# RajeshRk18/exacto

Hardware: AMD Instinct MI355X
Metric: ciphertext muls/sec (bfv_mul_and_relin) (higher is better)
Workload: dtype u64; 1 GPU; bfv_mul_and_relin, BASELINE configs[2]; ring_degree=4096, ct_limbs=3, limb_bits=60, plain_modulus=65537, gadget_base=65536, gadget_digits=12, batch_per_gpu=1024, global_batch=1024, parallelism=batch-shard x1

## Files before the change

### exacto_amd/csrc/context.hip

```cpp
#include <algorithm>
#include <array>
#include <cxxabi.h>
#include <dlfcn.h>
#include <chrono>
#include <condition_variable>
#include <cmath>
#include <cstdio>
#include <cstdlib>
#include <cstring>
#include <functional>
#include <map>
#include <memory>
#include <mutex>
#include <set>
#include <string>
#include <thread>
#include <type_traits>
#include <vector>

#include "../../include/exacto_hip.h"
#include "exacto_internal.hpp"

using namespace exacto;

// ... 3054 lines not shown


extern "C" int exacto_gen_galois_key_dev(exacto_ctx* c, const uint64_t* sk, uint64_t element, double sigma,
                                         const uint64_t* key, uint64_t stream, size_t num_keys, uint64_t* gk) {
    if (int e = check_ctx(c)) return e;
    if (!key || !sk || !gk) return invalid_param("null argument");
    if (num_keys == 0) return 0;
    const int n = c->n, L = c->L;
    const long Ln = (long)L * n;
    if (c->enc_buf.grow((size_t)(2 * n + Ln) * sizeof(u64))) return EXACTO_ERR_HIP;
    u64 *t0 = c->enc_buf, *t1 = t0 + n, *s_auto = t1 + n;
    HIP_TRY(dev_copy(t0, sk, n * sizeof(u64), c->stream));
    if (int e = run_ntt(c, contiguous(t0, 1, 1, 0, 1, n), 1, true)) return e;
    launch_automorph(t0, n, t1, n, 1, 1, n, 1, element, c->d_primes, 0, c->stream);
    launch_lift_q0(t1, s_auto, 1, n, L, c->d_primes, c->stream);
    CHECK_LAUNCH();
    if (int e = ntt_items(c, s_auto, 1, 0, L)) return e;
    std::vector<u64> gpow(num_keys * L);
    for (int l = 0; l < L; ++l) {
        const u64 q = c->primes[l];
        u64 g = 1 % q;
        const u64 b = c->gbase % q;
        for (size_t i = 0; i < num_keys; ++i) {
            gpow[i * L + l] = g;
            g = (u64)((u128)g * b % q);
        }
    }
    if (c->d_gpow.grow(gpow.size() * sizeof(u64))) return EXACTO_ERR_HIP;
    HIP_TRY(hipStreamSynchronize(c->stream));
    if (int e_ = upload(c, c->d_gpow, gpow.data(), gpow.size() * sizeof(u64))) return e_;
    const ChaChaKey k = chacha_key(key);
    if (int e = sample_polys(c, KG_UNIFORM, k, stream, gk + Ln, 2 * Ln, 0, 2, (long)num_keys, sigma)) return e;
    if (int e = sample_polys(c, KG_GAUSSIAN, k, stream, gk, 2 * Ln, 1, 2, (long)num_keys, sigma)) return e;
    if (int e = ntt_items(c, gk, (long)num_keys, 2 * Ln, 2L * L)) return e;
    launch_combine(KG_GALOIS, gk, (long)num_keys, 2 * Ln, Ln, sk, s_auto, nullptr, nullptr, c->d_gpow, n, L,
                   c->d_primes, c->stream);
    CHECK_LAUNCH();
    HIP_TRY(hipStreamSynchronize(c->stream));
    return 0;
}

extern "C" int exacto_bfv_apply_automorphism_dev(exacto_ctx* c, const uint64_t* ct, size_t polys, uint64_t element,
                                                 const uint64_t* gk, size_t num_keys, uint64_t* out, size_t B) {
    if (int e = check_ctx(c)) return e;
    if (polys != 2) return invalid_param("automorphism requires degree-1 ciphertext");
    if (num_keys == 0 || !gk) return invalid_param("galois key is empty");
    if (B == 0) return 0;
    const int n = c->n, L = c->L;
    const long Ln = (long)L * n;
    const int guse = (int)std::min<size_t>(c->G, num_keys);
    const size_t count = (size_t)guse * 2 * Ln;
    const bool d16 = c->digit16 && c->gbase <= 65536;
    const Ks32Basis& kb = c->kn;
    const bool k32 = d16 && c->ks32 && kb.S > 0 && c->path == EXACTO_PATH_EXACT_RNS;
    if (k32) {
        if (int e = ks32_convert_key(c, gk, (size_t)guse, c->d_gk_rs, kb.S, kb.d_p32, kb.mac_form)) return e;
    } else {
        if (c->gk_s.grow(count * sizeof(u64))) return EXACTO_ERR_HIP;
        launch_shoup_companions(gk, c->gk_s, (long)count, n, L, c->d_primes, c->stream);
        CHECK_LAUNCH();
    }
    const size_t C = std::min<size_t>(c->chunk, B);
    LanePass pass;
    if (int e = pass.begin(c, (long)((B + C - 1) / C), C)) return e;
    for (size_t s0 = 0; s0 < B; s0 += C) {
        const int cnt = (int)std::min(C, B - s0);
        LaneGuard lane = pass.chunk((long)(s0 / C));
        const u64* src = ct + s0 * 2 * Ln;
        u64* dst = out + s0 * 2 * Ln;
        NttBatch nb{};
        nb.src = src; nb.src_item_stride = 2 * Ln;
        nb.dst = c->ws.coefQ; nb.dst_item_stride = 2 * Ln;
        nb.ppi = 2 * L; nb.prime_base = 0; nb.period = L;
        if (int e = run_ntt(c, nb, (long)cnt * 2 * L, true)) return e;
        launch_automorph(c->ws.coefQ, 2 * Ln, c->ws.T, 2 * Ln, cnt, 2, n, L, element, c->d_primes, -1, c->stream);
        CHECK_LAUNCH();
        if (k32) {
            launch_decompose(c->ws.T + Ln, 2 * Ln, c->ws.D, guse, cnt, n, c->d_crt, c->d_primes, L, c->stream,
                             c->ws.D16);
            CHECK_LAUNCH();
            launch_rows(c->ws.T + Ln, 2 * Ln, nullptr, 0, Ln, cnt, c->stream);
            CHECK_LAUNCH();
            ks32_digits(c->ws.D16, c->ws.DS, cnt, guse, kb.S, c->logn, kb.d_p32, kb.mac_form, c->stream);
            ks32_mac(c->ws.DS, c->d_gk_rs, c->ws.U, cnt, guse, L, kb.S, n, kb.d_p32, kb.mac_form, c->stream);
            ks32_crt(c->ws.U, c->ws.T, 2 * Ln, cnt, L, kb.S, c->logn, kb.d_kst, kb.d_p32, c->d_primes, kb.mac_form, c->stream,
                     c->ks_fpc && kb.fpc_max >= 1);
            CHECK_LAUNCH();
            NttBatch rb{};
            rb.src = c->ws.T; rb.src_item_stride = 2 * Ln;
            rb.dst = dst; rb.dst_item_stride = 2 * Ln;
            rb.ppi = 2 * L; rb.prime_base = 0; rb.period = L;
            if (int e = run_ntt(c, rb, (long)cnt * 2 * L, false)) return e;
            continue;
        }
        NttBatch c0{};
        c0.src = c->ws.T; c0.src_item_stride = 2 * Ln;
        c0.dst = dst; c0.dst_item_stride = 2 * Ln;
        c0.ppi = L; c0.prime_base = 0; c0.period = L;
        if (int e = run_ntt(c, c0, (long)cnt * L, false)) return e;
        launch_rows(dst + Ln, 2 * Ln, nullptr, 0, Ln, cnt, c->stream);
        launch_decompose(c->ws.T + Ln, 2 * Ln, c->ws.D, guse, cnt, n, c->d_crt, c->d_primes, L, c->stream,
                         d16 ? c->ws.D16 : nullptr);
        CHECK_LAUNCH();
        NttBatch db = contiguous(c->ws.D, cnt, (long)guse * L, 0, L, n);
        if (d16) {
            db.src16 = c->ws.D16;
            db.src16_item_stride = (long)guse * n;
        }
        if (int e = run_ntt(c, db, (long)cnt * guse * L, false)) return e;
        launch_relin_mac(dst, 2 * Ln, c->ws.D, gk, c->gk_s, guse, dst, 2 * Ln, cnt, n, L, c->d_primes, c->stream);
        CHECK_LAUNCH();
    }
    return 0;
}

extern "C" int exacto_gen_galois_key(exacto_ctx* c, const uint64_t* sk, uint64_t element, double sigma,
                                     const uint64_t* key, uint64_t stream, size_t num_keys, uint64_t* gk) {
    if (!c) return invalid_param("null context");
    return host_call(c, {{sk, c->L * poly_bytes(c)}}, num_keys * 2 * c->L * poly_bytes(c), gk,
                     [&](std::vector<u64*>& d, u64* o) {
                         return exacto_gen_galois_key_dev(c, d[0], element, sigma, key, stream, num_keys, o);
                     });
}

extern "C" int exacto_bfv_apply_automorphism(exacto_ctx* c, const uint64_t* ct, size_t polys, uint64_t element,
                                             const uint64_t* gk, size_t num_keys, uint64_t* out, size_t B) {
    if (!c) return invalid_param("null context");
    if (polys != 2) return invalid_param("automorphism requires degree-1 ciphertext");
    return host_call(c, {{ct, B * 2 * c->L * poly_bytes(c)}, {gk, num_keys * 2 * c->L * poly_bytes(c)}},
                     B * 2 * c->L * poly_bytes(c), out, [&](std::vector<u64*>& d, u64* o) {
                         return exacto_bfv_apply_automorphism_dev(c, d[0], polys, element, d[1], num_keys, o, B);
                     });
}


static int pl_scratch(exacto_ctx* c, size_t words) {
    if (c->pl_buf.grow(words * sizeof(u64))) return EXACTO_ERR_HIP;
    return 0;
}

static int lift_plain(exacto_ctx* c, const u64* pt, long items, bool delta) {
    const long Ln = (long)c->L * c->n;
    if (delta)
        if (int e = delta_residues(c)) return e;
    if (int e = pl_scratch(c, (size_t)items * Ln)) return e;
    launch_scale_plain(pt, delta ? c->d_delta : nullptr, c->pl_buf, items, c->n, c->L, c->d_primes, c->stream);
    CHECK_LAUNCH();
    return ntt_items(c, c->pl_buf, items, Ln, c->L);
}

extern "C" int exacto_bfv_plain_mul_dev(exacto_ctx* c, const uint64_t* ct, size_t polys, const uint64_t* pt,
                                        uint64_t* out, size_t B) {
    if (int e = check_ctx(c)) return e;
    if (!ct || !pt || !out) return invalid_param("null argument");
    if (polys == 0) return invalid_param("ciphertext has no components");
    if (B == 0) return 0;
    if (int e = lift_plain(c, pt, (long)B, false)) return e;
    const long Ln = (long)c->L * c->n;
    launch_plain_apply(PLAIN_MUL, ct, (long)polys * Ln, out, (long)B, (int)polys, c->pl_buf, Ln, c->n, c->L, c->d_primes,
                       c->stream);
    CHECK_LAUNCH();
    return 0;
}

extern "C" int exacto_bfv_plain_add_dev(exacto_ctx* c, const uint64_t* ct, size_t polys, const uint64_t* pt,
                                        uint64_t* out, size_t B) {
    if (int e = check_ctx(c)) return e;
// ... 2227 lines not shown
```

### exacto_amd/csrc/exacto_internal.hpp

```cpp
#pragma once
#include "arith.hpp"

namespace exacto {

struct NttBatch {
    const u64* src;
    const u64* src_off;
    long src_item_stride;
    u64* dst;
    long dst_item_stride;
    int ppi;
    int prime_base;
    int period;
    const int16_t* src16;
    long src16_item_stride;
    int lazy_out;
};

enum class MulPath : int { Exact = 0, Hps = 1 };

struct CrtTables {
    int L;
    int K;
    int G;
    int gshift;
    u64 gbase;
    u64 plain;
    u64 gq_w[EXACTO_MAX_L][EXACTO_MAX_L];
    u64 gq_ws[EXACTO_MAX_L][EXACTO_MAX_L];
    u64 halfQ_mr[EXACTO_MAX_L];
    u64 qpref_w[EXACTO_MAX_L + 1][EXACTO_MAX_PRIMES];
    u64 qpref_ws[EXACTO_MAX_L + 1][EXACTO_MAX_PRIMES];
    u64 gp_w[EXACTO_MAX_K][EXACTO_MAX_K];
    u64 gp_ws[EXACTO_MAX_K][EXACTO_MAX_K];
    u64 halfP_mr[EXACTO_MAX_K];
    u64 ppref_w[EXACTO_MAX_K + 1][EXACTO_MAX_L];
    u64 ppref_ws[EXACTO_MAX_K + 1][EXACTO_MAX_L];
    u64 qinvp_w[EXACTO_MAX_K], qinvp_ws[EXACTO_MAX_K];
    u64 pq_w[EXACTO_MAX_K], pq_ws[EXACTO_MAX_K];
    u64 qpq_w[EXACTO_MAX_L + 1][EXACTO_MAX_K], qpq_ws[EXACTO_MAX_L + 1][EXACTO_MAX_K];
    u64 fpc_pq[EXACTO_MAX_K];
    u64 fpc_qpq[EXACTO_MAX_L][EXACTO_MAX_K];
    u64 fpc_neg[EXACTO_MAX_K];
    double fpc_inv[EXACTO_MAX_K];
    u64 fpc_pm[EXACTO_MAX_K][EXACTO_MAX_L];
    u64 fpc_negP[EXACTO_MAX_L];
    u64 fpq_pz_w[EXACTO_MAX_L], fpq_pz_ws[EXACTO_MAX_L];
    double fpq_inv0[EXACTO_MAX_L], fpq_inv1[EXACTO_MAX_L];
    u64 fpq_c[EXACTO_MAX_L][EXACTO_MAX_K];
    u64 fpq_qo_w[EXACTO_MAX_L], fpq_qo_ws[EXACTO_MAX_L];
    int near;
    int fast;
    int special;
    int digit_small;
    u64 pmod_w[EXACTO_MAX_PRIMES], pmod_ws[EXACTO_MAX_PRIMES];
    u64 Qwords[EXACTO_MAX_L];
    u64 hq[EXACTO_MAX_PRIMES];
    u64 hps_qinv[2];
    u64 hps_p1_inv_p0, hps_p0_inv_p1;
    u64 hps_pc;
    u64 hps_qinv_s[2];
    u64 hps_t_w[2], hps_t_ws[2];
    u64 hps_pq_w[2], hps_pq_ws[2];
    u64 hps_kPq[3];
    u64 hps_P[2], hps_halfP[2];
};

bool launch_ntt_fwd2(const NttBatch& nb1, int count1, const NttBatch& nb2, int count2, int logn,
                     const PrimeConst* primes, hipStream_t s);
void launch_ntt(const NttBatch& nb, int count, int logn, bool inverse, bool lazy, const PrimeConst* primes,
                hipStream_t s, bool asm_fwd = false, bool asm_inv = false, int qbits = 64);

void launch_shoup_companions(const u64* w, u64* ws, long count, int n, int L, const PrimeConst* primes,
                             hipStream_t s);

#define EXACTO_KS32_MAXS 4
struct Prime32 {
    uint32_t p;
    uint32_t n_inv, n_inv_s;
    uint32_t last_w, last_ws;
    uint32_t c32, c32s;
    uint32_t k63;
    uint32_t fn_inv, fn_inv_s;
    uint32_t flast_w, flast_ws;
    double inv_p;
    const uint2* tw_fwd;
    const uint2* tw_inv;
};
struct Ks32Tables {
    uint32_t ginv[EXACTO_KS32_MAXS][EXACTO_KS32_MAXS];
    uint32_t ginv_s[EXACTO_KS32_MAXS][EXACTO_KS32_MAXS];
    uint32_t halfP[EXACTO_KS32_MAXS];
    u64 pref_w[EXACTO_MAX_L][EXACTO_KS32_MAXS];
    u64 pref_ws[EXACTO_MAX_L][EXACTO_KS32_MAXS];
    u64 negP[EXACTO_MAX_L];
    uint32_t fpc_c[EXACTO_MAX_L][EXACTO_KS32_MAXS][2];
    uint32_t fpc_n[EXACTO_MAX_L][2];
};
void ks32_digits(const int16_t* D16, uint32_t* DS, int items, int G, int S, int logn, const Prime32* primes,
                 int form, hipStream_t st);
void ks32_digits32(const int32_t* D, uint32_t* DS, int items, int G, int S, int logn, const Prime32* primes,
                   int form, hipStream_t st);
void ks32_key(const u64* K, uint32_t* RS, long rows, int L, int S, int logn, const Prime32* primes,
              const PrimeConst* qprimes, int form, hipStream_t st);
void ks32_key_norms(const u64* K, u64* out, long rows, int L, int n, const PrimeConst* qprimes, hipStream_t st);
void ks32_mac(const uint32_t* DS, const uint32_t* RS, uint32_t* U, int items, int G, int L, int S, int n,
              const Prime32* primes, int mac_form, hipStream_t st);
void ks32_mac_hoist(const uint32_t* DS, const uint32_t* RSK, uint32_t* U, const uint32_t* perm,
                    const unsigned char* ident, int items, int R, int G, int L, int S, int n, const Prime32* primes,
                    int mac_form, hipStream_t st);
void ks32_crt(const uint32_t* U, u64* R, long r_stride, int items, int L, int S, int logn, const Ks32Tables* KT,
              const Prime32* primes, const PrimeConst* qprimes, int form, hipStream_t st, bool fpc = false);

struct BatchTab {
    Prime32 P;
    u64 mu;
    const uint32_t* perm;
};
enum { BF_STRICT = 3 };
void launch_batch_transform(bool encode, const u64* in, u64* out, long count, int logn, const BatchTab& tab, int form,
                            hipStream_t s);
void launch_dbfv_batch(bool encode, const u64* in, u64* out, long count, int d, u64 base, u64 p, int logn,
                       const BatchTab& tab, int form, hipStream_t s);

struct Operands {
    const u64* a;
    const u64* a_off;
    long a_stride;
    const u64* b;
    const u64* b_off;
    long b_stride;
    const u64* ea;
    const u64* ea_off;
    const u64* eb;
    const u64* eb_off;
};

bool launch_polymul(const u64* A, const u64* B, u64* out, long rows, int period, int logn, const PrimeConst* primes,
                    hipStream_t s);
void launch_mul_inv(const u64* A, const u64* B, u64* out, long rows, int period, int logn, bool lazy, bool asm_inv,
                    const PrimeConst* primes, hipStream_t s);
struct DropPrimeK {
    u64 w[EXACTO_MAX_L], ws[EXACTO_MAX_L];
};
void launch_drop_prime(const u64* in, u64* out, long rows, int l, bool round, const DropPrimeK& C, int logn, bool lazy,
                       bool asm_rounds, const PrimeConst* primes, hipStream_t s);
void launch_inv_tensor(const Operands& op, const u64* extP, u64* T, int items, int logn, int L, int K, bool lazy,
                       const PrimeConst* primes, hipStream_t s, bool asm_inv = false, bool p2only = false,
                       int qbits = 64, int share_np = 0, bool lazy_out = false, bool fold = false,
                       bool square = false);
bool crt_fold_tensor_ok(int logn, bool asm_inv, bool lazy_out);
void launch_phase(const u64* ct, int polys, long ct_stride, const u64* sk, u64* out, int items, int n, int L,
                  const PrimeConst* primes, hipStream_t s);
void launch_decrypt_round(const u64* X, u64* out, int items, int n, int L, const CrtTables* ct,
                          const PrimeConst* primes, u64 plain, hipStream_t s);
int noise_chunks(int n);
void launch_noise(const u64* X, const u64* expected, u64* plain_out, u64* part, u64* out, long items, int group,
                  int n, int L, const CrtTables* ct, const PrimeConst* primes, const u64* delta, u64 plain,
                  bool round, hipStream_t s);
void launch_dbfv_recompose(const u64* digits, u64* out, int items, int n, int d, u64 base, u64 plain, u64 t,
                           bool scalar, hipStream_t s);
void launch_exact_lift(const u64* coefQ, u64* extP, long rows, int n, const CrtTables* ct,
                       const PrimeConst* primes, int L, int K, int mode, hipStream_t s);
void launch_hps_extend(const u64* coefQ, u64* extP, long rows, int n, const PrimeConst* primes,
                       int K, hipStream_t s);
bool exact_scale_sp_ok(int L, int K, int mode);
void launch_exact_scale(const u64* T, u64* R, long r_stride, int ncomp_r, u64* D, int16_t* D16, int guse,
                        int items, int n, const CrtTables* ct, const PrimeConst* primes, int L,
                        int K, int mode, hipStream_t s, int gshift = -1, bool c2only = false,
                        bool digits8 = false, bool fpc = false, double fpq_lim = 0.0, bool fold = false);
bool exact_scale_fold_ok(int L, int K, int mode, bool fpc, double fpq_lim);
void launch_hps_scale(const u64* T, u64* R, long r_stride, int ncomp_r, u64* D, void* D16, bool d8, int guse,
                      int items, int n, const CrtTables* ct, const PrimeConst* primes, int K, bool fast,
                      hipStream_t s);
void launch_decompose(const u64* C2, long c2_stride, u64* D, int guse, int items, int n,
                      const CrtTables* ct, const PrimeConst* primes, int L, hipStream_t s, int16_t* D16 = nullptr);
void launch_rows(u64* dst, long dst_stride, const u64* src, long src_stride, long len, long rows, hipStream_t s);
void launch_copy_u64(u64* dst, const u64* src, long words, hipStream_t s);
void launch_xcd_probe(const u64* src, u64* dst, long words, uint32_t* xcc, int blocks, hipStream_t s);
void launch_fill_u32(uint32_t* dst, uint32_t v, long words, hipStream_t s);
void debug_watch_set(const void* lo, const void* hi, uint32_t* hit, hipStream_t s = nullptr);
void launch_relin_mac(const u64* base, long base_stride, const u64* D, const u64* rlk, const u64* rlk_s,
                      int guse, u64* out, long out_stride, int items, int n, int L, const PrimeConst* primes,
                      hipStream_t s);

void launch_hoist_mac(bool lt, const u64* ct, const u64* D, const u64* keys, const u64* keys_s, const uint32_t* perm,
                      const unsigned char* ident, const u64* pts, u64* out, int R, int guse, int items, int n, int L,
                      const PrimeConst* primes, hipStream_t s);
void launch_hoist_c0(const u64* ct, const uint32_t* perm, const unsigned char* ident, u64* H, int R, int items, int n,
                     int L, const PrimeConst* primes, hipStream_t s);
// ... 102 lines not shown
```

### exacto_amd/csrc/ks32.hip

```cpp
#include "exacto_internal.hpp"
#include "ks32_dev.hpp"

#include <algorithm>

namespace exacto {


template <int LOGN, typename DT, int FORM>
__global__ void __launch_bounds__((1 << LOGN) / 16)
ks32_digit_ntt_kernel(const DT* __restrict__ D16, uint32_t* __restrict__ DS, int G, int S,
                      const Prime32* __restrict__ primes) {
    constexpr int N = 1 << LOGN, T = N / 16;
    __shared__ uint32_t lds[N];
    const int tid = threadIdx.x;
    const uint32_t b = blockIdx.x;
    const int s = (int)(b % (uint32_t)S);
    const long ig = b / (uint32_t)S;
    const Prime32& P = primes[s];
    const DT* src = D16 + ig * N;
    uint32_t x[16];
    constexpr bool SIN = FORM == F32_LAZY && sizeof(DT) == 2;
#pragma unroll
    for (int k = 0; k < 16; ++k) {
        const int d = src[tid + k * T];
        x[k] = SIN ? (uint32_t)d : d < 0 ? P.p + (uint32_t)d : (uint32_t)d;
    }
    fwd32_store<LOGN, FORM, SIN, FORM != F32_LAZY>(x, lds, tid, P, DS + (long)b * N);
}

template <int LOGN, int FORM>
__global__ void __launch_bounds__((1 << LOGN) / 16)
ks32_key_kernel(const u64* __restrict__ K, uint32_t* __restrict__ RS, int L, int S,
                const Prime32* __restrict__ primes, const PrimeConst* __restrict__ qprimes) {
    constexpr int N = 1 << LOGN, T = N / 16;
    __shared__ uint32_t lds[N];
    const int tid = threadIdx.x;
    const uint32_t b = blockIdx.x;
    const int s = (int)(b % (uint32_t)S);
    const uint32_t row = b / (uint32_t)S;
    const int l = (int)(row % (uint32_t)L);
    const Prime32& P = primes[s];
    const u64 q = qprimes[l].q, half = q >> 1;
    const u64* src = K + (long)row * N;
    uint32_t x[16];
#pragma unroll
    for (int k = 0; k < 16; ++k) {
        const u64 r = src[tid + k * T];
        if (r > half) {
            const uint32_t m = (uint32_t)((q - r) % P.p);
            x[k] = m == 0 ? 0 : P.p - m;
        } else {
            x[k] = (uint32_t)(r % P.p);
        }
    }
    fwd32_store<LOGN, FORM>(x, lds, tid, P, RS + (long)b * N);
}

__global__ void __launch_bounds__(256)
ks32_key_norm_kernel(const u64* __restrict__ K, u64* __restrict__ out, int L, int n,
                     const PrimeConst* __restrict__ qprimes) {
    __shared__ u64 part[256];
    const uint32_t row = blockIdx.x;
    const u64 q = qprimes[row % (uint32_t)L].q, half = q >> 1;
    const u64* src = K + (long)row * n;
    u64 acc = 0;
    for (int j = threadIdx.x; j < n; j += 256) {
        const u64 r = src[j];
        acc += (r > half ? q - r : r) >> 20;
    }
    part[threadIdx.x] = acc;
    __syncthreads();
    for (int w = 128; w > 0; w >>= 1) {
        if ((int)threadIdx.x < w) part[threadIdx.x] += part[threadIdx.x + w];
        __syncthreads();
    }
    if (threadIdx.x == 0) out[row] = part[0];
}

__device__ __forceinline__ uint32_t red_s64(long long x, const Prime32& P) {
    const uint32_t p = P.p;
    const uint32_t hu = (uint32_t)((unsigned long long)x >> 32) ^ 0x80000000u;
    const uint32_t a = red32(shoup32(hu, P.c32, P.c32s, p), p);
    const uint32_t b = red32(red32((uint32_t)x, 2 * p), p);
    return red32(red32(a + b, p) + P.k63, p);
}

__device__ __forceinline__ uint32_t red_s64_lz(long long x, const Prime32& P) {
    const uint32_t p = P.p;
    const uint32_t hu = (uint32_t)((unsigned long long)x >> 32) ^ 0x80000000u;
    const uint32_t a = red32(shoup32(hu, P.c32, P.c32s, p), p);
    const uint32_t lo = (uint32_t)x;
    const uint32_t b = lo - (lo >> 30) * p;
    const uint32_t s = a + b + P.k63;
    return min(s, s - 2 * p);
}

__device__ __forceinline__ long long red_s64_lazy(long long x, const Prime32& P) {
    const uint32_t hu = (uint32_t)((unsigned long long)x >> 32) ^ 0x80000000u;
    const uint32_t a = shoup32(hu, P.c32, P.c32s, P.p);
    return (long long)((unsigned long long)a + (uint32_t)x + P.k63);
}

constexpr int KS_LS = 64;
template <int CLB, int NW, int RUN, bool LZ = false>
__global__ void __launch_bounds__(NW * 64)
ks32_mac_kernel(const int* __restrict__ DS, const int* __restrict__ RS, uint32_t* __restrict__ U,
                int G, int CL, int S, int items, int n, const Prime32* __restrict__ primes) {
    extern __shared__ int kl[];
    constexpr int IG = 4 * NW;
    const int lane = threadIdx.x & (KS_LS - 1);
    const int wave = __builtin_amdgcn_readfirstlane(threadIdx.x / KS_LS);
    const int nb = n / KS_LS;
    const int jb = blockIdx.x % nb;
    const int s = (blockIdx.x / nb) % S;
    const int cl0 = (blockIdx.x / (nb * S)) * CLB;
    const int j = jb * KS_LS + lane;
    const Prime32& P = primes[s];
    for (int rr = wave; rr < G * CLB; rr += NW) {
        const int g = rr / CLB, c = rr - g * CLB;
        kl[rr * KS_LS + lane] = RS[(((long)g * CL + cl0 + c) * S + s) * n + jb * KS_LS + lane];
    }
    __syncthreads();
    const int it_end = min(items, (int)(blockIdx.y + 1) * IG);
    for (int it = blockIdx.y * IG + wave; it < it_end; it += NW) {
        const int* dp = DS + ((long)it * G * S + s) * n + j;
        long long acc[CLB];
#pragma unroll
        for (int c = 0; c < CLB; ++c) acc[c] = 0;
        for (int g0 = 0; g0 < G; g0 += RUN) {
            int d[RUN];
#pragma unroll
            for (int e = 0; e < RUN; ++e) d[e] = dp[(long)min(g0 + e, G - 1) * S * n];
#pragma unroll
            for (int e = 0; e < RUN; ++e) d[e] = g0 + e < G ? d[e] : 0;
#pragma unroll
            for (int e = 0; e < RUN; ++e) {
                const int* kg = kl + (min(g0 + e, G - 1) * CLB) * KS_LS + lane;
#pragma unroll
                for (int c = 0; c < CLB; ++c) acc[c] += (long long)d[e] * kg[c * KS_LS];
            }
            if (g0 + RUN < G) {
#pragma unroll
                for (int c = 0; c < CLB; ++c) acc[c] = red_s64_lazy(acc[c], P);
            }
        }
#pragma unroll
        for (int c = 0; c < CLB; ++c)
            U[(((long)it * CL + cl0 + c) * S + s) * n + j] = LZ ? red_s64_lz(acc[c], P) : red_s64(acc[c], P);
    }
}

template <int CLB, int NW, int RUN, bool LZ = false>
__global__ void __launch_bounds__(NW * 64)
ks32_mac_hoist_kernel(const int* __restrict__ DS, const int* __restrict__ RSK, uint32_t* __restrict__ U,
                      const uint32_t* __restrict__ perm, const unsigned char* __restrict__ ident, int G, int CL, int S,
                      int items, int n, const Prime32* __restrict__ primes) {
    extern __shared__ int kl[];
    constexpr int IG = 4 * NW;
    const int lane = threadIdx.x & (KS_LS - 1);
    const int wave = __builtin_amdgcn_readfirstlane(threadIdx.x / KS_LS);
    const int nb = n / KS_LS;
    const int jb = blockIdx.x % nb;
    const int s = (blockIdx.x / nb) % S;
    const int cl0 = (blockIdx.x / (nb * S)) * CLB;
    const int r = blockIdx.z, R = gridDim.z;
    const int j = jb * KS_LS + lane;
    const Prime32& P = primes[s];
    const int it_end = min(items, (int)(blockIdx.y + 1) * IG);
    if (ident[r]) {
        for (int it = blockIdx.y * IG + wave; it < it_end; it += NW)
#pragma unroll
            for (int c = 0; c < CLB; ++c) U[((((long)it * R + r) * CL + cl0 + c) * S + s) * n + j] = 0;
        return;
    }
    const int* RS = RSK + (long)r * G * CL * S * n;
    for (int rr = wave; rr < G * CLB; rr += NW) {
        const int g = rr / CLB, c = rr - g * CLB;
        kl[rr * KS_LS + lane] = RS[(((long)g * CL + cl0 + c) * S + s) * n + jb * KS_LS + lane];
    }
    __syncthreads();
    const int pj = (int)perm[(long)r * n + j];
    for (int it = blockIdx.y * IG + wave; it < it_end; it += NW) {
        const int* dp = DS + ((long)it * G * S + s) * n + pj;
        long long acc[CLB];
#pragma unroll
        for (int c = 0; c < CLB; ++c) acc[c] = 0;
        for (int g0 = 0; g0 < G; g0 += RUN) {
            int d[RUN];
#pragma unroll
            for (int e = 0; e < RUN; ++e) d[e] = dp[(long)min(g0 + e, G - 1) * S * n];
#pragma unroll
            for (int e = 0; e < RUN; ++e) d[e] = g0 + e < G ? d[e] : 0;
#pragma unroll
            for (int e = 0; e < RUN; ++e) {
                const int* kg = kl + (min(g0 + e, G - 1) * CLB) * KS_LS + lane;
#pragma unroll
                for (int c = 0; c < CLB; ++c) acc[c] += (long long)d[e] * kg[c * KS_LS];
            }
            if (g0 + RUN < G) {
#pragma unroll
                for (int c = 0; c < CLB; ++c) acc[c] = red_s64_lazy(acc[c], P);
            }
        }
#pragma unroll
        for (int c = 0; c < CLB; ++c)
            U[((((long)it * R + r) * CL + cl0 + c) * S + s) * n + j] = LZ ? red_s64_lz(acc[c], P) : red_s64(acc[c], P);
    }
}

template <int LOGN, int S, bool LAZY, bool FPC>
__global__ void __launch_bounds__((1 << LOGN) / 16)
ks32_crt_kernel(const uint32_t* __restrict__ U, u64* __restrict__ R, long r_stride, int L,
                const Ks32Tables* __restrict__ KT, const Prime32* __restrict__ primes,
                const PrimeConst* __restrict__ qprimes) {
    constexpr int N = 1 << LOGN, T = N / 16;
    __shared__ uint32_t lds[N];
    const int tid = threadIdx.x;
    const uint32_t b = blockIdx.x;
    u64 x[16];
    ks32_crt_values<LOGN, S, LAZY, FPC>(x, U, R, r_stride, L, b, lds, tid, KT, primes, qprimes);
    const uint32_t CL = 2 * L;
    const long item = b / CL;
    const __amdgpu_buffer_rsrc_t rd = poly_rsrc(R + item * r_stride + (long)(b - (uint32_t)item * CL) * N, N * 8);
#pragma unroll
    for (int k = 0; k < 16; ++k) buf_st64(rd, x[k], tid * 8, k * T * 8);
}

template <typename OT, typename IT>
__global__ void __launch_bounds__(256)
ks32_digit_sum_kernel(const IT* __restrict__ D, int npairs, const int* __restrict__ term_start,
                      const CombineTerm* __restrict__ terms, OT* __restrict__ out, int d, int gu, int n,
                      int nsh) {
    const uint32_t row = blockIdx.x >> nsh;
    const int j = (int)(blockIdx.x & ((1u << nsh) - 1)) * 2048 + 8 * threadIdx.x;
    const uint32_t g = row % (uint32_t)gu;
    const uint32_t ik = row / (uint32_t)gu;
    const int k = (int)(ik % (uint32_t)d);
    const long item = ik / (uint32_t)d;
    int acc[8] = {0, 0, 0, 0, 0, 0, 0, 0};
    for (int t = term_start[k]; t < term_start[k + 1]; ++t) {
        const IT* src = D + ((item * npairs + terms[t].pair) * gu + g) * (long)n + j;
        if constexpr (sizeof(IT) == 2) {
            const uint4 w = *reinterpret_cast<const uint4*>(src);
            const uint32_t v[4] = {w.x, w.y, w.z, w.w};
#pragma unroll
            for (int h = 0; h < 4; ++h) {
                acc[2 * h] += (int)(int16_t)(v[h] & 0xFFFF);
                acc[2 * h + 1] += (int)(int16_t)(v[h] >> 16);
            }
        } else {
            const uint2 w = *reinterpret_cast<const uint2*>(src);
            const uint32_t v[2] = {w.x, w.y};
#pragma unroll
            for (int h = 0; h < 8; ++h) acc[h] += (int)(int8_t)(v[h >> 2] >> (8 * (h & 3)));
        }
    }
    if constexpr (sizeof(OT) == 2) {
        uint4 o;
        uint32_t* op = &o.x;
#pragma unroll
        for (int h = 0; h < 4; ++h) op[h] = ((uint32_t)acc[2 * h] & 0xFFFF) | ((uint32_t)acc[2 * h + 1] << 16);
        *reinterpret_cast<uint4*>(out + (long)row * n + j) = o;
    } else {
        int4* o4 = reinterpret_cast<int4*>(out + (long)row * n + j);
        o4[0] = make_int4(acc[0], acc[1], acc[2], acc[3]);
        o4[1] = make_int4(acc[4], acc[5], acc[6], acc[7]);
    }
}


#define FORM_SWITCH(form, CALL)                          \
    switch (form) {                                      \
        case F32_LAZY: CALL(F32_LAZY); break;            \
        case F32_NARROW: CALL(F32_NARROW); break;        \
        default: CALL(F32_WIDE); break;                  \
    }

template <int LOGN>
static void ks32_launch_digits(const void* D, bool wide, uint32_t* DS, int items, int G, int S, const Prime32* primes,
                               int form, hipStream_t st) {
    const dim3 grid((unsigned)((long)items * G * S)), block((1 << LOGN) / 16);
#define DIG_(F_)                                                                                                \
    do {                                                                                                        \
        if (wide)                                                                                               \
            EXACTO_LAUNCH((ks32_digit_ntt_kernel<LOGN, int32_t, F_>), grid, block, 0, st, (const int32_t*)D, \
                               DS, G, S, primes);                                                               \
        else                                                                                                    \
            EXACTO_LAUNCH((ks32_digit_ntt_kernel<LOGN, int16_t, F_>), grid, block, 0, st, (const int16_t*)D, \
                               DS, G, S, primes);                                                               \
    } while (0)
    FORM_SWITCH(form, DIG_)
#undef DIG_
}

template <int LOGN>
static void ks32_launch_key(const u64* K, uint32_t* RS, long rows, int L, int S, const Prime32* primes,
                            const PrimeConst* qprimes, int form, hipStream_t st) {
#define KEY_(F_) EXACTO_LAUNCH((ks32_key_kernel<LOGN, F_>), dim3((unsigned)(rows * S)), dim3((1 << LOGN) / 16), 0, \
                                    st, K, RS, L, S, primes, qprimes)
    FORM_SWITCH(form, KEY_)
#undef KEY_
}

template <int LOGN, bool LAZY>
static void ks32_launch_crt(const uint32_t* U, u64* R, long r_stride, int items, int L, int S, const Ks32Tables* KT,
                            const Prime32* primes, const PrimeConst* qprimes, hipStream_t st, bool fpc) {
    const dim3 grid((unsigned)((long)items * 2 * L)), block((1 << LOGN) / 16);
#define CRT_(S_, F_) EXACTO_LAUNCH((ks32_crt_kernel<LOGN, S_, LAZY, F_>), grid, block, 0, st, U, R, r_stride, L, KT, \
                                   primes, qprimes)
    if (S == 2) {
        if (fpc) CRT_(2, true); else CRT_(2, false);
    } else if (S == 3) {
        if (fpc) CRT_(3, true); else CRT_(3, false);
    } else {
        if (fpc) CRT_(4, true); else CRT_(4, false);
    }
#undef CRT_
}

#define KS32_SWITCH(logn, CALL)                  \
    switch (logn) {                              \
        case 10: CALL(10); break;                \
        case 11: CALL(11); break;                \
        case 12: CALL(12); break;                \
        case 13: CALL(13); break;                \
        case 14: CALL(14); break;                \
        default: break;                          \
    }

void ks32_digits(const int16_t* D16, uint32_t* DS, int items, int G, int S, int logn, const Prime32* primes, int form,
                 hipStream_t st) {
    if (items <= 0) return;
#define CALL(L_) ks32_launch_digits<L_>(D16, false, DS, items, G, S, primes, form, st)
    KS32_SWITCH(logn, CALL)
#undef CALL
}

void ks32_digits32(const int32_t* D, uint32_t* DS, int items, int G, int S, int logn, const Prime32* primes, int form,
                   hipStream_t st) {
    if (items <= 0) return;
#define CALL(L_) ks32_launch_digits<L_>(D, true, DS, items, G, S, primes, form, st)
    KS32_SWITCH(logn, CALL)
#undef CALL
}

void ks32_key(const u64* K, uint32_t* RS, long rows, int L, int S, int logn, const Prime32* primes,
              const PrimeConst* qprimes, int form, hipStream_t st) {
    if (rows <= 0) return;
#define CALL(L_) ks32_launch_key<L_>(K, RS, rows, L, S, primes, qprimes, form, st)
    KS32_SWITCH(logn, CALL)
#undef CALL
}

void ks32_key_norms(const u64* K, u64* out, long rows, int L, int n, const PrimeConst* qprimes, hipStream_t st) {
    if (rows <= 0) return;
    EXACTO_LAUNCH(ks32_key_norm_kernel, dim3((unsigned)rows), dim3(256), 0, st, K, out, L, n, qprimes);
}

void ks32_mac(const uint32_t* DS, const uint32_t* RS, uint32_t* U, int items, int G, int L, int S, int n,
              const Prime32* primes, int mac_form, hipStream_t st) {
    if (items <= 0) return;
    const int CL = 2 * L;
    int CLB = CL;
    while (CLB > 1 && (CL % CLB != 0 || (size_t)G * CLB * KS_LS * sizeof(int) > 65536)) --CLB;
    const size_t lds = (size_t)G * CLB * KS_LS * sizeof(int);
    const int NW = lds > 32768 ? 8 : 4;
    const dim3 grid((unsigned)((n / KS_LS) * S * (CL / CLB)), (unsigned)((items + 4 * NW - 1) / (4 * NW)));
    const int* ds = reinterpret_cast<const int*>(DS);
    const int* rs = reinterpret_cast<const int*>(RS);
#define MAC_(C_, W_, R_, Z_) EXACTO_LAUNCH((ks32_mac_kernel<C_, W_, R_, Z_>), grid, dim3(W_ * 64), lds, st, ds, rs, U, G, CL, S, items, n, primes)
#define MAC(C_)                                                  \
    do {                                                         \
        if (mac_form == 2) { if (NW == 8) MAC_(C_, 8, 12, true); else MAC_(C_, 4, 12, true); } \
        else if (mac_form == 1) { if (NW == 8) MAC_(C_, 8, 12, false); else MAC_(C_, 4, 12, false); } \
        else { if (NW == 8) MAC_(C_, 8, 7, false); else MAC_(C_, 4, 7, false); }          \
    } while (0)
    switch (CLB) {
        case 8: MAC(8); break;
        case 6: MAC(6); break;
        case 4: MAC(4); break;
        case 3: MAC(3); break;
        case 2: MAC(2); break;
        default: MAC(1); break;
    }
#undef MAC
#undef MAC_
}

void ks32_mac_hoist(const uint32_t* DS, const uint32_t* RSK, uint32_t* U, const uint32_t* perm,
                    const unsigned char* ident, int items, int R, int G, int L, int S, int n, const Prime32* primes,
                    int mac_form, hipStream_t st) {
    if (items <= 0 || R <= 0) return;
    const int CL = 2 * L;
    int CLB = CL;
    while (CLB > 1 && (CL % CLB != 0 || (size_t)G * CLB * KS_LS * sizeof(int) > 65536)) --CLB;
    const size_t lds = (size_t)G * CLB * KS_LS * sizeof(int);
    const int NW = lds > 32768 ? 8 : 4;
    const dim3 grid((unsigned)((n / KS_LS) * S * (CL / CLB)), (unsigned)((items + 4 * NW - 1) / (4 * NW)), (unsigned)R);
    const int* ds = reinterpret_cast<const int*>(DS);
    const int* rs = reinterpret_cast<const int*>(RSK);
#define MAC_(C_, W_, R_, Z_) EXACTO_LAUNCH((ks32_mac_hoist_kernel<C_, W_, R_, Z_>), grid, dim3(W_ * 64), lds, st, ds, rs, U, perm, ident, G, CL, S, items, n, primes)
#define MAC(C_)                                                  \
    do {                                                         \
        if (mac_form == 2) { if (NW == 8) MAC_(C_, 8, 12, true); else MAC_(C_, 4, 12, true); } \
        else if (mac_form == 1) { if (NW == 8) MAC_(C_, 8, 12, false); else MAC_(C_, 4, 12, false); } \
        else { if (NW == 8) MAC_(C_, 8, 7, false); else MAC_(C_, 4, 7, false); }          \
    } while (0)
    switch (CLB) {
        case 8: MAC(8); break;
        case 6: MAC(6); break;
        case 4: MAC(4); break;
        case 3: MAC(3); break;
        case 2: MAC(2); break;
        default: MAC(1); break;
    }
#undef MAC
#undef MAC_
}

void ks32_digit_sum(const void* D, bool in8, int npairs, const int* term_start, const CombineTerm* terms, void* out,
                    bool wide, int items, int d, int gu, int n, hipStream_t st) {
    const long rows = (long)items * d * gu;
    if (rows <= 0) return;
    const int nb = n >= 2048 ? n / 2048 : 1;
    const dim3 grid((unsigned)(rows * nb)), block(n >= 2048 ? 256 : n / 8);
    const int nsh = __builtin_ctz((unsigned)nb);
#define DSUM_(OT, IT) EXACTO_LAUNCH((ks32_digit_sum_kernel<OT, IT>), grid, block, 0, st, (const IT*)D, npairs, \
                                         term_start, terms, (OT*)out, d, gu, n, nsh)
    if (wide) {
        if (in8) DSUM_(int32_t, int8_t); else DSUM_(int32_t, int16_t);
    } else {
        if (in8) DSUM_(int16_t, int8_t); else DSUM_(int16_t, int16_t);
    }
#undef DSUM_
}

void ks32_crt(const uint32_t* U, u64* R, long r_stride, int items, int L, int S, int logn, const Ks32Tables* KT,
              const Prime32* primes, const PrimeConst* qprimes, int form, hipStream_t st, bool fpc) {
    if (items <= 0) return;
    fpc = fpc && (S <= 3 || form != F32_WIDE);
#define CALL(L_)                                                                                                \
    do {                                                                                                        \
        if (form == F32_LAZY) ks32_launch_crt<L_, true>(U, R, r_stride, items, L, S, KT, primes, qprimes, st, fpc); \
        else ks32_launch_crt<L_, false>(U, R, r_stride, items, L, S, KT, primes, qprimes, st, fpc);                \
    } while (0)
    KS32_SWITCH(logn, CALL)
#undef CALL
}

}
```

Measured before the change: 482,800 bfv_mul_and_relin/s.

## Add vectorized, software-pipelined ks32 MAC kernel and XCD-aware digit NTT block remap

Rewrites the key-switch MAC kernel so it can process V coefficients per lane with vector loads and software-pipeline the next digit run's loads behind the current multiply-accumulates. It also remaps digit-NTT block indices so consecutive primes of one item are grouped per XCD, and replaces a division with a reciprocal multiply-high. The automorphism call site explicitly passes wide=false, so only the default-wide callers (e.g. relinearization in bfv_mul) get the new path. The wide path may need more than 64KB LDS and raises the attribute, which risks lower occupancy.

```diff
diff --git a/exacto_amd/csrc/context.hip b/exacto_amd/csrc/context.hip
--- a/exacto_amd/csrc/context.hip
+++ b/exacto_amd/csrc/context.hip
@@ -3160,7 +3160,7 @@
             launch_rows(c->ws.T + Ln, 2 * Ln, nullptr, 0, Ln, cnt, c->stream);
             CHECK_LAUNCH();
             ks32_digits(c->ws.D16, c->ws.DS, cnt, guse, kb.S, c->logn, kb.d_p32, kb.mac_form, c->stream);
-            ks32_mac(c->ws.DS, c->d_gk_rs, c->ws.U, cnt, guse, L, kb.S, n, kb.d_p32, kb.mac_form, c->stream);
+            ks32_mac(c->ws.DS, c->d_gk_rs, c->ws.U, cnt, guse, L, kb.S, n, kb.d_p32, kb.mac_form, c->stream, false);
             ks32_crt(c->ws.U, c->ws.T, 2 * Ln, cnt, L, kb.S, c->logn, kb.d_kst, kb.d_p32, c->d_primes, kb.mac_form, c->stream,
                      c->ks_fpc && kb.fpc_max >= 1);
             CHECK_LAUNCH();
diff --git a/exacto_amd/csrc/exacto_internal.hpp b/exacto_amd/csrc/exacto_internal.hpp
--- a/exacto_amd/csrc/exacto_internal.hpp
+++ b/exacto_amd/csrc/exacto_internal.hpp
@@ -105,7 +105,7 @@
               const PrimeConst* qprimes, int form, hipStream_t st);
 void ks32_key_norms(const u64* K, u64* out, long rows, int L, int n, const PrimeConst* qprimes, hipStream_t st);
 void ks32_mac(const uint32_t* DS, const uint32_t* RS, uint32_t* U, int items, int G, int L, int S, int n,
-              const Prime32* primes, int mac_form, hipStream_t st);
+              const Prime32* primes, int mac_form, hipStream_t st, bool wide = true);
 void ks32_mac_hoist(const uint32_t* DS, const uint32_t* RSK, uint32_t* U, const uint32_t* perm,
                     const unsigned char* ident, int items, int R, int G, int L, int S, int n, const Prime32* primes,
                     int mac_form, hipStream_t st);
diff --git a/exacto_amd/csrc/ks32.hip b/exacto_amd/csrc/ks32.hip
--- a/exacto_amd/csrc/ks32.hip
+++ b/exacto_amd/csrc/ks32.hip
@@ -5,19 +5,27 @@
 
 namespace exacto {
 
+
+#ifndef EXACTO_KS32_DIGIT_XCD
+#define EXACTO_KS32_DIGIT_XCD 1
+#endif
 
 template <int LOGN, typename DT, int FORM>
 __global__ void __launch_bounds__((1 << LOGN) / 16)
 ks32_digit_ntt_kernel(const DT* __restrict__ D16, uint32_t* __restrict__ DS, int G, int S,
-                      const Prime32* __restrict__ primes) {
+                      const Prime32* __restrict__ primes, uint32_t s_inv, uint32_t full) {
     constexpr int N = 1 << LOGN, T = N / 16;
     __shared__ uint32_t lds[N];
     const int tid = threadIdx.x;
-    const uint32_t b = blockIdx.x;
-    const int s = (int)(b % (uint32_t)S);
-    const long ig = b / (uint32_t)S;
+    uint32_t b = blockIdx.x;
+    if (EXACTO_KS32_DIGIT_XCD && b < full) {
+        const uint32_t x = b & 7, slot = b >> 3, q = __umulhi(slot, s_inv);
+        b = (q * 8 + x) * (uint32_t)S + (slot - q * (uint32_t)S);
+    }
+    const uint32_t ig = EXACTO_KS32_DIGIT_XCD ? __umulhi(b, s_inv) : b / (uint32_t)S;
+    const int s = (int)(b - ig * (uint32_t)S);
     const Prime32& P = primes[s];
-    const DT* src = D16 + ig * N;
+    const DT* src = D16 + (long)ig * N;
     uint32_t x[16];
     constexpr bool SIN = FORM == F32_LAZY && sizeof(DT) == 2;
 #pragma unroll
@@ -102,51 +110,152 @@
 }
 
 constexpr int KS_LS = 64;
-template <int CLB, int NW, int RUN, bool LZ = false>
+#ifndef EXACTO_KS32_MAC_WIDE
+#define EXACTO_KS32_MAC_WIDE 1
+#endif
+#ifndef EXACTO_KS32_MAC_V
+#define EXACTO_KS32_MAC_V 2
+#endif
+#ifndef EXACTO_KS32_MAC_NW
+#define EXACTO_KS32_MAC_NW 8
+#endif
+#ifndef EXACTO_KS32_MAC_IPW
+#define EXACTO_KS32_MAC_IPW 4
+#endif
+
+template <int V> struct KsVec { typedef int T __attribute__((ext_vector_type(V))); };
+template <> struct KsVec<1> { typedef int T; };
+template <int V>
+__device__ __forceinline__ void ks_ld(int (&o)[V], const int* p) {
+    if constexpr (V == 1) o[0] = *p;
+    else {
+        const typename KsVec<V>::T w = *reinterpret_cast<const typename KsVec<V>::T*>(p);
+#pragma unroll
+        for (int v = 0; v < V; ++v) o[v] = w[v];
+    }
+}
+template <int V>
+__device__ __forceinline__ void ks_st(int* p, const int (&x)[V]) {
+    if constexpr (V == 1) *p = x[0];
+    else {
+        typename KsVec<V>::T w;
+#pragma unroll
+        for (int v = 0; v < V; ++v) w[v] = x[v];
+        *reinterpret_cast<typename KsVec<V>::T*>(p) = w;
+    }
+}
+
+template <int CLB, int NW, int RUN, bool LZ = false, int V = 1, int IPW = 4, bool PIPE = false>
 __global__ void __launch_bounds__(NW * 64)
 ks32_mac_kernel(const int* __restrict__ DS, const int* __restrict__ RS, uint32_t* __restrict__ U,
                 int G, int CL, int S, int items, int n, const Prime32* __restrict__ primes) {
+    static_assert(PIPE || V == 1, "the form before the wide lanes: one coefficient per lane");
     extern __shared__ int kl[];
-    constexpr int IG = 4 * NW;
+    constexpr int IG = IPW * NW;
+    constexpr int LS = KS_LS * V;
     const int lane = threadIdx.x & (KS_LS - 1);
     const int wave = __builtin_amdgcn_readfirstlane(threadIdx.x / KS_LS);
-    const int nb = n / KS_LS;
+    const int nb = n / LS;
     const int jb = blockIdx.x % nb;
     const int s = (blockIdx.x / nb) % S;
     const int cl0 = (blockIdx.x / (nb * S)) * CLB;
-    const int j = jb * KS_LS + lane;
+    const int j = jb * LS + lane * V;
     const Prime32& P = primes[s];
-    for (int rr = wave; rr < G * CLB; rr += NW) {
-        const int g = rr / CLB, c = rr - g * CLB;
-        kl[rr * KS_LS + lane] = RS[(((long)g * CL + cl0 + c) * S + s) * n + jb * KS_LS + lane];
+    const int it_end = min(items, (int)(blockIdx.y + 1) * IG);
+    const long gs = (long)S * n;
+    auto load_run = [&](int (&d)[RUN][V], int it, int g0) {
+        const int* dp = DS + ((long)it * G * S + s) * n + j;
+#pragma unroll
+        for (int e = 0; e < RUN; ++e) ks_ld<V>(d[e], dp + (long)min(g0 + e, G - 1) * gs);
+    };
+    long long acc[CLB][V];
+    auto mac_digit = [&](int (&d)[V], int g) {
+#pragma unroll
+        for (int v = 0; v < V; ++v) d[v] = g < G ? d[v] : 0;
+        const int* kg = kl + (min(g, G - 1) * CLB) * LS + lane * V;
+#pragma unroll
+        for (int c = 0; c < CLB; ++c) {
+            int k[V];
+            ks_ld<V>(k, kg + c * LS);
+#pragma unroll
+            for (int v = 0; v < V; ++v) acc[c][v] += (long long)d[v] * k[v];
+        }
+    };
+    auto mac_run = [&](int (&d)[RUN][V], int g0) {
+#pragma unroll
+        for (int e = 0; e < RUN; ++e) mac_digit(d[e], g0 + e);
+    };
+    auto lazy_run = [&]() {
+#pragma unroll
+        for (int c = 0; c < CLB; ++c)
+#pragma unroll
+            for (int v = 0; v < V; ++v) acc[c][v] = red_s64_lazy(acc[c][v], P);
+    };
+    auto store_item = [&](int it) {
+#pragma unroll
+        for (int c = 0; c < CLB; ++c) {
+            int r[V];
+#pragma unroll
+            for (int v = 0; v < V; ++v) r[v] = (int)(LZ ? red_s64_lz(acc[c][v], P) : red_s64(acc[c][v], P));
+            ks_st<V>(reinterpret_cast<int*>(U) + (((long)it * CL + cl0 + c) * S + s) * n + j, r);
+        }
+    };
+    auto clear = [&]() {
+#pragma unroll
+        for (int c = 0; c < CLB; ++c)
+#pragma unroll
+            for (int v = 0; v < V; ++v) acc[c][v] = 0;
+    };
+    int it = blockIdx.y * IG + wave, g0 = 0;
+    int da[RUN][V];
+    if constexpr (PIPE) {
+        if (it < it_end) load_run(da, it, 0);
+    }
+    if constexpr (PIPE) {
+        for (int g = wave; g < G; g += NW) {
+            int k[CLB][V];
+#pragma unroll
+            for (int c = 0; c < CLB; ++c) ks_ld<V>(k[c], RS + (((long)g * CL + cl0 + c) * S + s) * n + j);
+#pragma unroll
+            for (int c = 0; c < CLB; ++c) ks_st<V>(kl + (g * CLB + c) * LS + lane * V, k[c]);
+        }
+    } else {
+        for (int rr = wave; rr < G * CLB; rr += NW) {
+            const int g = rr / CLB, c = rr - g * CLB;
+            kl[rr * KS_LS + lane] = RS[(((long)g * CL + cl0 + c) * S + s) * n + jb * KS_LS + lane];
+        }
     }
     __syncthreads();
-    const int it_end = min(items, (int)(blockIdx.y + 1) * IG);
-    for (int it = blockIdx.y * IG + wave; it < it_end; it += NW) {
-        const int* dp = DS + ((long)it * G * S + s) * n + j;
-        long long acc[CLB];
-#pragma unroll
-        for (int c = 0; c < CLB; ++c) acc[c] = 0;
-        for (int g0 = 0; g0 < G; g0 += RUN) {
-            int d[RUN];
-#pragma unroll
-            for (int e = 0; e < RUN; ++e) d[e] = dp[(long)min(g0 + e, G - 1) * S * n];
-#pragma unroll
-            for (int e = 0; e < RUN; ++e) d[e] = g0 + e < G ? d[e] : 0;
+    if constexpr (!PIPE) {
+        for (; it < it_end; it += NW) {
+            clear();
+            for (g0 = 0; g0 < G; g0 += RUN) {
+                load_run(da, it, g0);
+                mac_run(da, g0);
+                if (g0 + RUN < G) lazy_run();
+            }
+            store_item(it);
+        }
+    } else {
+        clear();
+        while (it < it_end) {
+            int ng = g0 + RUN, nit = it;
+            if (ng >= G) { ng = 0; nit = it + NW; }
+            if (nit >= it_end) {
+                mac_run(da, g0);
+                store_item(it);
+                break;
+            }
+            const int* np = DS + ((long)nit * G * S + s) * n + j;
 #pragma unroll
             for (int e = 0; e < RUN; ++e) {
-                const int* kg = kl + (min(g0 + e, G - 1) * CLB) * KS_LS + lane;
-#pragma unroll
-                for (int c = 0; c < CLB; ++c) acc[c] += (long long)d[e] * kg[c * KS_LS];
+                mac_digit(da[e], g0 + e);
+                ks_ld<V>(da[e], np + (long)min(ng + e, G - 1) * gs);
             }
-            if (g0 + RUN < G) {
-#pragma unroll
-                for (int c = 0; c < CLB; ++c) acc[c] = red_s64_lazy(acc[c], P);
-            }
-        }
-#pragma unroll
-        for (int c = 0; c < CLB; ++c)
-            U[(((long)it * CL + cl0 + c) * S + s) * n + j] = LZ ? red_s64_lz(acc[c], P) : red_s64(acc[c], P);
+            if (ng != 0) lazy_run();
+            else { store_item(it); clear(); }
+            it = nit; g0 = ng;
+        }
     }
 }
 
@@ -280,14 +389,15 @@
 static void ks32_launch_digits(const void* D, bool wide, uint32_t* DS, int items, int G, int S, const Prime32* primes,
                                int form, hipStream_t st) {
     const dim3 grid((unsigned)((long)items * G * S)), block((1 << LOGN) / 16);
+    const uint32_t s_inv = (uint32_t)((1ull << 32) / (unsigned)S) + 1, full = grid.x / (8u * S) * (8u * S);
 #define DIG_(F_)                                                                                                \
     do {                                                                                                        \
         if (wide)                                                                                               \
             EXACTO_LAUNCH((ks32_digit_ntt_kernel<LOGN, int32_t, F_>), grid, block, 0, st, (const int32_t*)D, \
-                               DS, G, S, primes);                                                               \
+                               DS, G, S, primes, s_inv, full);                                                               \
         else                                                                                                    \
             EXACTO_LAUNCH((ks32_digit_ntt_kernel<LOGN, int16_t, F_>), grid, block, 0, st, (const int16_t*)D, \
-                               DS, G, S, primes);                                                               \
+                               DS, G, S, primes, s_inv, full);                                                               \
     } while (0)
     FORM_SWITCH(form, DIG_)
 #undef DIG_
@@ -357,23 +467,82 @@
     EXACTO_LAUNCH(ks32_key_norm_kernel, dim3((unsigned)rows), dim3(256), 0, st, K, out, L, n, qprimes);
 }
 
+struct Ks32MacShape {
+    int V, NW, IPW, CLB;
+    bool wide;
+    size_t lds;
+};
+
+static int ks32_mac_clb(int G, int CL, int V, size_t cap) {
+    int CLB = CL;
+    while (CLB > 1 && (CL % CLB != 0 || (size_t)G * CLB * KS_LS * V * sizeof(int) > cap)) --CLB;
+    return CLB;
+}
+
+static Ks32MacShape ks32_mac_shape(int n, int G, int CL, int S, int items, bool aligned16) {
+    (void)S; (void)items;
+    Ks32MacShape sh;
+    sh.V = 1;
+    sh.CLB = ks32_mac_clb(G, CL, 1, 65536);
+    sh.IPW = 4;
+    sh.wide = false;
+    sh.lds = (size_t)G * sh.CLB * KS_LS * sizeof(int);
+    sh.NW = sh.lds > 32768 ? 8 : 4;
+    constexpr int WV = EXACTO_KS32_MAC_V;
+    if (EXACTO_KS32_MAC_WIDE && aligned16 && n % (KS_LS * WV) == 0 && ks32_mac_clb(G, CL, WV, 81920) == sh.CLB) {
+        sh.wide = true;
+        sh.V = WV;
+        sh.NW = EXACTO_KS32_MAC_NW;
+        sh.IPW = EXACTO_KS32_MAC_IPW;
+        sh.lds *= WV;
+    }
+    return sh;
+}
+
+template <int C_, int W_, int R_, bool Z_, int V_, int I_, bool P_>
+static void ks32_mac_launch(dim3 grid, size_t lds, hipStream_t st, const int* ds, const int* rs, uint32_t* U, int G,
+                            int CL, int S, int items, int n, const Prime32* primes) {
+    if (lds > 65536) {
+        static bool raised[64] = {};
+        int dev = 0;
+        (void)hipGetDevice(&dev);
+        if (dev >= 0 && dev < 64 && !raised[dev]) {
+            raised[dev] = hipFuncSetAttribute(reinterpret_cast<const void*>(&ks32_mac_kernel<C_, W_, R_, Z_, V_, I_, P_>),
+                                              hipFuncAttributeMaxDynamicSharedMemorySize, 81920) == hipSuccess;
+        }
+    }
+    EXACTO_LAUNCH((ks32_mac_kernel<C_, W_, R_, Z_, V_, I_, P_>), grid, dim3(W_ * 64), lds, st, ds, rs, U, G, CL, S, items,
+                  n, primes);
+}
+
 void ks32_mac(const uint32_t* DS, const uint32_t* RS, uint32_t* U, int items, int G, int L, int S, int n,
-              const Prime32* primes, int mac_form, hipStream_t st) {
+              const Prime32* primes, int mac_form, hipStream_t st, bool wide) {
     if (items <= 0) return;
     const int CL = 2 * L;
-    int CLB = CL;
-    while (CLB > 1 && (CL % CLB != 0 || (size_t)G * CLB * KS_LS * sizeof(int) > 65536)) --CLB;
-    const size_t lds = (size_t)G * CLB * KS_LS * sizeof(int);
-    const int NW = lds > 32768 ? 8 : 4;
-    const dim3 grid((unsigned)((n / KS_LS) * S * (CL / CLB)), (unsigned)((items + 4 * NW - 1) / (4 * NW)));
+    const bool aligned16 = ((reinterpret_cast<uintptr_t>(DS) | reinterpret_cast<uintptr_t>(RS) |
+                             reinterpret_cast<uintptr_t>(U)) & 15) == 0;
+    const Ks32MacShape sh = ks32_mac_shape(n, G, CL, S, items, aligned16 && wide);
+    const bool pipe = EXACTO_KS32_MAC_WIDE != 0 && wide;
+    const int CLB = sh.CLB, IG = sh.IPW * sh.NW;
+    const dim3 grid((unsigned)((n / (KS_LS * sh.V)) * S * (CL / CLB)), (unsigned)((items + IG - 1) / IG));
     const int* ds = reinterpret_cast<const int*>(DS);
     const int* rs = reinterpret_cast<const int*>(RS);
-#define MAC_(C_, W_, R_, Z_) EXACTO_LAUNCH((ks32_mac_kernel<C_, W_, R_, Z_>), grid, dim3(W_ * 64), lds, st, ds, rs, U, G, CL, S, items, n, primes)
+#define MAC_(C_, W_, R_, Z_, V_, I_, P_) \
+    ks32_mac_launch<C_, W_, R_, Z_, V_, I_, P_>(grid, sh.lds, st, ds, rs, U, G, CL, S, items, n, primes)
+#define MAC_F(C_, R_, Z_)                                                                                          \
+    do {                                                                                                           \
+        if (sh.wide)                                                                                               \
+            MAC_(C_, EXACTO_KS32_MAC_NW, R_, Z_, EXACTO_KS32_MAC_V, EXACTO_KS32_MAC_IPW, true);                    \
+        else if (pipe && sh.NW == 8) MAC_(C_, 8, R_, Z_, 1, 4, (EXACTO_KS32_MAC_WIDE != 0));                       \
+        else if (pipe) MAC_(C_, 4, R_, Z_, 1, 4, (EXACTO_KS32_MAC_WIDE != 0));                                     \
+        else if (sh.NW == 8) MAC_(C_, 8, R_, Z_, 1, 4, false);                                                     \
+        else MAC_(C_, 4, R_, Z_, 1, 4, false);                                                                     \
+    } while (0)
 #define MAC(C_)                                                  \
     do {                                                         \
-        if (mac_form == 2) { if (NW == 8) MAC_(C_, 8, 12, true); else MAC_(C_, 4, 12, true); } \
-        else if (mac_form == 1) { if (NW == 8) MAC_(C_, 8, 12, false); else MAC_(C_, 4, 12, false); } \
-        else { if (NW == 8) MAC_(C_, 8, 7, false); else MAC_(C_, 4, 7, false); }          \
+        if (mac_form == 2) MAC_F(C_, 12, true);                  \
+        else if (mac_form == 1) MAC_F(C_, 12, false);            \
+        else MAC_F(C_, 7, false);                                \
     } while (0)
     switch (CLB) {
         case 8: MAC(8); break;
@@ -384,6 +553,7 @@
         default: MAC(1); break;
     }
 #undef MAC
+#undef MAC_F
 #undef MAC_
 }
 
```

Result: no change. 485,400 bfv_mul_and_relin/s, median of 6 (+0.6%).
